# microsoft/YOLaT-VectorGraphicsRecognition

Hardware: AMD Instinct MI355X
Metric: graphs_per_sec (higher is better)
Workload: dtype f32

## Files before the change

yolat_vectorgraphicsrecognition_amd/csrc/common.hpp:

```cpp
#pragma once
#include <hip/hip_runtime.h>
#include <stdint.h>

#include "../../include/yolat_hip.h"

typedef float f32x16 __attribute__((ext_vector_type(16)));
typedef float f32x4 __attribute__((ext_vector_type(4)));

#define YL_LAUNCH_CHECK()                          \
  do {                                             \
    hipError_t e__ = hipGetLastError();            \
    if (e__ != hipSuccess) return (int)e__;        \
  } while (0)

static inline int yl_cdiv(long a, long b) { return (int)((a + b - 1) / b); }
static inline bool yl_aligned16(const void* p) { return (((uintptr_t)p) & 15) == 0; }
static inline bool yl_strict_fp32() {
  static int v = -1;
  if (v < 0) { const char* e = getenv("YOLAT_STRICT_FP32"); v = (e && e[0] == '1') ? 1 : 0; }
  return v != 0;
}

struct YlGate { const int* p; int val; };
__device__ __forceinline__ bool yl_gate_dead(const YlGate& g) { return g.p != nullptr && *g.p != g.val; }
// ... 542 lines not shown
    }
    __syncthreads();
  }

  static_assert(TM <= 2 && TN <= 2, "epilogue expansion covers up to 2x2 sub-tiles");
#define YL_EPI(i, j)                                                                                              \
  if constexpr ((i) < TM && (j) < TN)                                                                             \
    wave_epilogue(acc[i][j], row0 + wm * WM + (i) * 32, col0 + wn * WN + (j) * 32 + l31, lhi, ep, M, N, pre[i][j], \
                  smem + wave * (32 * YL_STAGE_LD));
  YL_EPI(0, 0) YL_EPI(0, 1) YL_EPI(1, 0) YL_EPI(1, 1)
#undef YL_EPI
}

template <int BM, int BN, int BK, class AL, class BL, bool B_NFAST>
__global__ void __launch_bounds__(256) k_gemm_nt(AL A, BL B, Epilogue ep, int M, int N, int K) {
  int rt_, ct_;
  yl_xcd_tile(rt_, ct_);
  gemm_nt_tile<BM, BN, BK, AL, BL, B_NFAST>(A, B, ep, M, N, K, rt_, ct_);
}

template <int BM, int BN, int BK, class AL, class BL>
__global__ void __launch_bounds__(256) k_gemm_nt_pair(AL A0, BL B0, Epilogue e0, AL A1, BL B1, Epilogue e1,
                                                      int M, int N, int K) {
  if (blockIdx.y == 0) gemm_nt_tile<BM, BN, BK, AL, BL, false>(A0, B0, e0, M, N, K, blockIdx.x, 0);
  else gemm_nt_tile<BM, BN, BK, AL, BL, false>(A1, B1, e1, M, N, K, blockIdx.x, 0);
}

static __global__ void __launch_bounds__(256) k_gemm_nt_two(DenseOp A0, DenseOp B0, Epilogue e0, int M0, int N0, int K0, int tm0,
                                                     int tn0, DenseOp A1, DenseOp B1, Epilogue e1, int M1, int N1,
                                                     int K1, int tm1, int tn1) {
  const int n1 = tm1 * tn1, n1p = (n1 + 7) & ~7;
  const int id = blockIdx.x;
  if (id < n1p) {
    if (id < n1) gemm_nt_tile<64, 64, 32, DenseOp, DenseOp, false>(A1, B1, e1, M1, N1, K1, id / tn1, id % tn1);
    return;
  }
  const int n0 = tm0 * tn0, j = id - n1p;
  const int chunk = n0 >> 3, rem = n0 & 7;
  const int xcd = j & 7, slot = j >> 3;
  const int logical = xcd * chunk + (xcd < rem ? xcd : rem) + slot;
  gemm_nt_tile<64, 64, 32, DenseOp, DenseOp, false>(A0, B0, e0, M0, N0, K0, logical / tn0, logical % tn0);
}

struct NodeUv {
  DenseOp af, wuv, wr, as, wn;
  Epilogue euv, er, en;
  int N, C, Cin;
};
int yl_build_node_uv(NodeUv* a, const float* f_in, int64_t ld_f, const float* s_in, int64_t ld_s, int64_t N,
                     int64_t Cin, const float* Wuv, const float* uv_bias, const float* Wr, const float* br,
                     const float* Wn, const float* bn, const float* sn, const float* tn, int64_t C, float* UV,
                     int64_t ld_uv, float* f_out, int64_t ld_fo, float* s_out, int64_t ld_so);
constexpr int N3_KMAX = 8, N3_ROWS = 32, N3_ITERS = 4;
template <int WAVES = 4, int ITERS = N3_ITERS>
__device__ __forceinline__ void node3_smallk_body(const NodeUv& a, int vb) {
  constexpr int ROWS = 8 * WAVES;
  __shared__ __attribute__((aligned(16))) float xs[ITERS][WAVES][2][64];
  const int lane = threadIdx.x & 63, wave = threadIdx.x >> 6;
  const int C = a.C, Cin = a.Cin, N = a.N;
  const int r0 = vb * (ROWS * ITERS), r1 = yl_min(r0 + ROWS * ITERS, N);
  const int c4 = 4 * lane;
  const int prob = c4 < 2 * C ? 0 : (c4 < 3 * C ? 1 : 2);
  const int col = prob == 0 ? c4 : (prob == 1 ? c4 - 2 * C : c4 - 3 * C);
  const int relu = prob == 0 ? a.euv.relu : (prob == 1 ? a.er.relu : a.en.relu);
  float* Y = prob == 0 ? a.euv.Y : (prob == 1 ? a.er.Y : a.en.Y);
  unsigned short* Yh = prob == 0 ? a.euv.Yh : (prob == 1 ? a.er.Yh : a.en.Yh);
  const long ldy = prob == 0 ? a.euv.ldy : (prob == 1 ? a.er.ldy : a.en.ldy);
  const int lu = lane >> 3, lk = lane & 7;
  float fa[ITERS], sa[ITERS];
#pragma unroll
  for (int it = 0; it < ITERS; ++it) {
    const long row = yl_min(r0 + ROWS * it + 8 * wave + lu, N - 1);
    const int kc = yl_min(lk, Cin - 1);
    const float f = a.af.p[row * a.af.ld + kc], g = a.as.p[row * a.as.ld + kc];
    fa[it] = lk < Cin ? f : 0.f;
    sa[it] = lk < Cin ? g : 0.f;
  }
  __shared__ __attribute__((aligned(16))) float wl[256][N3_KMAX];
  __shared__ float cl[3][256];
  if (threadIdx.x < 256) {
    const int t = threadIdx.x;
    const int tp = t < 2 * C ? 0 : (t < 3 * C ? 1 : 2);
    const int tc = tp == 0 ? t : (tp == 1 ? t - 2 * C : t - 3 * C);
    const float* __restrict__ twp = tp == 0 ? a.wuv.p : (tp == 1 ? a.wr.p : a.wn.p);
    const long tld = tp == 0 ? a.wuv.ld : (tp == 1 ? a.wr.ld : a.wn.ld);
    const float* tb = tp == 0 ? a.euv.bias : (tp == 1 ? a.er.bias : a.en.bias);
    const float* ts = tp == 0 ? a.euv.scale : (tp == 1 ? a.er.scale : a.en.scale);
    const float* th = tp == 0 ? a.euv.shift : (tp == 1 ? a.er.shift : a.en.shift);
    float wr_[N3_KMAX];
#pragma unroll
    for (int k = 0; k < N3_KMAX; ++k) wr_[k] = twp[(long)tc * tld + yl_min(k, Cin - 1)];
    const float vb_ = (tb ? tb : twp)[tb ? tc : 0], vs_ = (ts ? ts : twp)[ts ? tc : 0], vh_ = (ts ? th : twp)[ts ? tc : 0];
#pragma unroll
    for (int k = 0; k < N3_KMAX; ++k) wl[t][k] = k < Cin ? wr_[k] : 0.f;
    cl[0][t] = tb ? vb_ : 0.f;
    cl[1][t] = ts ? vs_ : 1.f;
    cl[2][t] = ts ? vh_ : 0.f;
  }
#pragma unroll
  for (int it = 0; it < ITERS; ++it) { xs[it][wave][0][lane] = fa[it]; xs[it][wave][1][lane] = sa[it]; }
  __syncthreads();
  float w[4][N3_KMAX], b[4], sc[4], sh[4];
#pragma unroll
  for (int j = 0; j < 4; ++j) {
    const float4 w0 = *reinterpret_cast<const float4*>(&wl[c4 + j][0]), w1 = *reinterpret_cast<const float4*>(&wl[c4 + j][4]);
    w[j][0] = w0.x; w[j][1] = w0.y; w[j][2] = w0.z; w[j][3] = w0.w;
    w[j][4] = w1.x; w[j][5] = w1.y; w[j][6] = w1.z; w[j][7] = w1.w;
    b[j] = cl[0][c4 + j]; sc[j] = cl[1][c4 + j]; sh[j] = cl[2][c4 + j];
  }
  const float floor = relu ? 0.f : -INFINITY;
#pragma unroll 1
  for (int it = 0; it < ITERS; ++it) {
    const float* mine = xs[it][wave][prob == 2 ? 1 : 0];
    const int rb = r0 + ROWS * it + 8 * wave;
    if (rb >= r1) break;
#pragma unroll
    for (int u = 0; u < 8; ++u) {
      const float4 x0 = *reinterpret_cast<const float4*>(mine + 8 * u);
      const float4 x1 = *reinterpret_cast<const float4*>(mine + 8 * u + 4);
      const float x[8] = {x0.x, x0.y, x0.z, x0.w, x1.x, x1.y, x1.z, x1.w};
      float v[4];
#pragma unroll
      for (int j = 0; j < 4; ++j) {
        float acc = 0.f;
#pragma unroll
        for (int k = 0; k < N3_KMAX; ++k) acc = fmaf(x[k], w[j][k], acc);
        v[j] = fmaxf(fmaf(acc + b[j], sc[j], sh[j]), floor);
      }
      const int row = rb + u;
      if (row < r1) {
        if (Yh != nullptr) {
          uint2 o;
          o.x = yl_pack_bf16(v[0], v[1]); o.y = yl_pack_bf16(v[2], v[3]);
          *reinterpret_cast<uint2*>(Yh + (long)row * ldy + col) = o;
        } else {
          *reinterpret_cast<float4*>(Y + (long)row * ldy + col) = make_float4(v[0], v[1], v[2], v[3]);
        }
      }
    }
  }
}

bool yl_node3_smallk_ok(const NodeUv& a);
bool yl_node3_smallk_shape_ok(const NodeUv& a);
int yl_node3_smallk(const NodeUv& a, hipStream_t st, YlGate gate = YlGate{nullptr, 0});
int yl_fusion_rows_x6_key64(const float* A, long lda, long N, long K, const float* W, const float* bias, long F,
                            const float* sgn, const int* node_seg, unsigned long long* keys, uint16_t* wsplit,
                            yolat_stream_t stream);
int yl_fusion_rows_bf16_key64(const float* A, long lda, long N, long K, const float* W, const float* bias, long F,
                              const float* sgn, const int* node_seg, unsigned long long* keys, uint16_t* wimg,
                              yolat_stream_t stream);
#define YL_POOL_ZERO 1
#define YL_POOL_MAX 2
#define YL_POOL_MEAN 4
struct PoolRider {
  const float* feats; const float* fsup; long ld; int D, F, P; const int* seg_ptr; float* Z; long ldz;
  int parts, blocks;
};
__device__ __forceinline__ void yl_pool_rider(const PoolRider& r, int vb, int nvb, int tid, int nthreads) {
  const int wz = (r.parts & YL_POOL_ZERO) ? r.F : 0, wx = (r.parts & YL_POOL_MAX) ? r.D : 0,
            wm = (r.parts & YL_POOL_MEAN) ? r.D : 0;
  const int W = wz + wx + wm;
  const long total = (long)r.P * W;
  for (long i = (long)vb * nthreads + tid; i < total; i += (long)nvb * nthreads) {
    const int p = (int)(i / W), c = (int)(i - (long)p * W);
    float* z = r.Z + (long)p * r.ldz;
    if (c < wz) { z[c] = 0.f; continue; }
    const bool is_max = c < wz + wx;
    const int k = is_max ? c - wz : c - wz - wx;
    const float* src = (is_max ? r.feats : r.fsup) + k;
    const int r0 = r.seg_ptr[p], r1 = r.seg_ptr[p + 1];
    float best = 0.f, sm = 0.f;
    bool any = false;
    int q = r0;
    for (; q + 8 <= r1; q += 8) {
      float v[8];
#pragma unroll
      for (int j = 0; j < 8; ++j) v[j] = src[(long)(q + j) * r.ld];
#pragma unroll
      for (int j = 0; j < 8; ++j) {
        if (!any || v[j] > best) { best = v[j]; any = true; }
        sm += v[j];
      }
    }
    for (; q < r1; ++q) {
      const float v = src[(long)q * r.ld];
      if (!any || v > best) { best = v; any = true; }
      sm += v;
    }
    if (is_max) z[r.F + k] = best;
    else {
      const int cnt = r1 - r0;
      z[2 * r.F + r.D + k] = sm / (float)(cnt > 1 ? cnt : 1);
// ... 443 lines not shown
```

yolat_vectorgraphicsrecognition_amd/csrc/graph.hip:

```cpp
#include "common.hpp"

__global__ void k_edge_count(const int64_t* edge, long se, long sc, int E, int N, int* src32,
                             int* dst32, int* cnt, int* status) {
  const int e = blockIdx.x * blockDim.x + threadIdx.x;
  if (e >= E) return;
  int64_t s = edge[(long)e * se];
  int64_t d = edge[(long)e * se + sc];
  if (s < 0 || s >= N || d < 0 || d >= N) {
    atomicOr(status, YOLAT_STATUS_EDGE_RANGE);
    s = s < 0 ? 0 : (s >= N ? N - 1 : s);
    d = d < 0 ? 0 : (d >= N ? N - 1 : d);
  }
  src32[e] = (int)s; dst32[e] = (int)d;
  atomicAdd(&cnt[d], 1);
}

__global__ void k_count32(const int* key, int n, int* cnt) {
  const int i = blockIdx.x * blockDim.x + threadIdx.x;
  if (i >= n) return;
  const int k = key[i];
  if (k >= 0) atomicAdd(&cnt[k], 1);
}

__global__ void __launch_bounds__(1024) k_scan_excl(int* cnt, int N, int* ptr) {
// ... 332 lines not shown
  const int d = dst32[e];
  items[local[d] + prep_prefix(btot, d / PREP_BLK) + rank[e]] = e;
}

__device__ __forceinline__ void prep_rows_body(int t, const int* local, const int* btot, int N, int E, const int* items,
                                               const int* src32, const int* dst32, const float4* attr, int* row_ptr,
                                               int* perm, int* src_csr, int* dst_csr, float4* attr_csr) {
  __shared__ int sh[PREP_OFFS + 4], wsum[4];
  const bool have = prep_offsets_lds(btot, (N + 1 + PREP_BLK - 1) / PREP_BLK, sh, wsum);
  auto off = [&](int i) { return local[i] + (have ? sh[i / PREP_BLK] : prep_prefix(btot, i / PREP_BLK)); };
  if (t <= N) row_ptr[t] = off(t);
  if (t >= E) return;
  const int e = items[t];
  const int i = dst32[e];
  const int b = off(i), en = off(i + 1);
  int r = 0;
  for (int j = b; j < en; j += 8) {
    int v[8];
#pragma unroll
    for (int k = 0; k < 8; ++k) v[k] = items[yl_min(j + k, en - 1)];
#pragma unroll
    for (int k = 0; k < 8; ++k) r += (j + k < en && v[k] < e) ? 1 : 0;
  }
  const int pos = b + r;
  const int sv = src32[e];
  const float4 av = attr[e];
  perm[pos] = e;
  src_csr[pos] = sv;
  dst_csr[pos] = i;
  attr_csr[pos] = av;
}

__global__ void __launch_bounds__(256) k_prep_rows(const int* local, const int* btot, int N, int E, const int* items,
                                                   const int* src32, const int* dst32, const float4* attr, int* row_ptr,
                                                   int* perm, int* src_csr, int* dst_csr, float4* attr_csr) {
  prep_rows_body(blockIdx.x * 256 + threadIdx.x, local, btot, N, E, items, src32, dst32, attr, row_ptr, perm, src_csr,
                 dst_csr, attr_csr);
}

template <int BK>
__global__ void __launch_bounds__(256) k_prep_rows_node3(const int* local, const int* btot, int N, int E,
                                                         const int* items, const int* src32, const int* dst32,
                                                         const float4* attr, int* row_ptr, int* perm, int* src_csr,
                                                         int* dst_csr, float4* attr_csr, int rows_blocks, NodeUv a) {
  if ((int)blockIdx.x < rows_blocks) {
    prep_rows_body(blockIdx.x * 256 + threadIdx.x, local, btot, N, E, items, src32, dst32, attr, row_ptr, perm, src_csr,
                   dst_csr, attr_csr);
    return;
  }
  const int t = blockIdx.x - rows_blocks;
  node_uv_tile<BK>(a, t >> 2, t & 3);
}

#define PS_T 1024
#define PS_NW (PS_T / 64)
#define PS_RMAX 256
#define PS_CAP 4096
#define PS_PF 8
#ifndef PS_NODE_ITERS
#define PS_NODE_ITERS 2
#endif
struct PrepSmall {
  const int64_t* edge; long se, sc; const float4* attr; const int64_t* bbox; long P;
  int E, N, R, nprep, nseg;
  int* row_ptr; int* perm; int* src_csr; int* dst_csr; float4* attr_csr; int* seg_ptr; int* node_seg; int* status;
};

__device__ __forceinline__ void ps_emit(const PrepSmall& g, int e, int d, int pos) {
  int64_t s = g.edge[(long)e * g.se];
  const float4 av = g.attr[e];
  if (s < 0 || s >= g.N) {
    atomicOr(g.status, YOLAT_STATUS_EDGE_RANGE);
    s = s < 0 ? 0 : g.N - 1;
  }
  g.perm[pos] = e;
  g.src_csr[pos] = (int)s;
  g.dst_csr[pos] = d;
  g.attr_csr[pos] = av;
}

template <int MODE>
__device__ __forceinline__ void ps_walk(const PrepSmall& g, int r0, int r1, int* rowcnt, int* cw, unsigned long long* mw,
                                        int* list_n, unsigned* list, int& below, int base, const int* rowstart) {
  const int lane = threadIdx.x & 63, w = threadIdx.x >> 6;
  const unsigned long long lt = (1ull << lane) - 1ull;
  const int per = ((g.E + PS_NW * 64 - 1) / (PS_NW * 64)) * 64;
  const int wb = w * per, we = yl_min(wb + per, g.E);
  for (int eb = wb; eb < we; eb += 64 * PS_PF) {
    int64_t dv[PS_PF];
#pragma unroll
    for (int j = 0; j < PS_PF; ++j) {
      const int e = yl_min(eb + 64 * j + lane, g.E - 1);
      dv[j] = g.edge[(long)e * g.se + g.sc];
    }
    if (MODE == 0) {
      unsigned long long om[PS_PF];
      int nown = 0;
#pragma unroll
      for (int j = 0; j < PS_PF; ++j) {
        const bool valid = eb + 64 * j + lane < we;
        const int d = dv[j] < 0 ? 0 : (dv[j] >= g.N ? g.N - 1 : (int)dv[j]);
        below += (valid && d < r0) ? 1 : 0;
        om[j] = __ballot(valid && d >= r0 && d < r1);
        nown += __popcll(om[j]);
      }
      if (nown == 0) continue;
      int s0 = 0;
      if (lane == 0) s0 = atomicAdd(list_n, nown);
      s0 = __builtin_amdgcn_readfirstlane(s0);
#pragma unroll
      for (int j = 0; j < PS_PF; ++j) {
        if ((om[j] >> lane) & 1ull) {
          const int dl = (dv[j] < 0 ? 0 : (dv[j] >= g.N ? g.N - 1 : (int)dv[j])) - r0, slot = s0 + __popcll(om[j] & lt);
          atomicAdd(&rowcnt[dl], 1);
          if (dv[j] < 0 || dv[j] >= g.N) atomicOr(g.status, YOLAT_STATUS_EDGE_RANGE);
          if (slot < PS_CAP) list[slot] = (unsigned)(eb + 64 * j + lane) | ((unsigned)dl << 20);
        }
        s0 += __popcll(om[j]);
      }
    } else {
#pragma unroll
      for (int j = 0; j < PS_PF; ++j) {
        const int e = eb + 64 * j + lane;
        const int d = dv[j] < 0 ? 0 : (dv[j] >= g.N ? g.N - 1 : (int)dv[j]);
        const bool own = e < we && d >= r0 && d < r1;
        if (__ballot(own) == 0ull) continue;
        const int dl = own ? d - r0 : 0;
        const int c = cw[dl];
        if (own) atomicOr(&mw[dl], 1ull << lane);
        const unsigned long long m = mw[dl];
        if (own && (m & lt) == 0ull) {
          cw[dl] = c + __popcll(m);
          mw[dl] = 0ull;
        }
        if (MODE == 2 && own) ps_emit(g, e, d, base + rowstart[dl] + c + __popcll(m & lt));
      }
    }
  }
}

__global__ void __launch_bounds__(PS_T) k_prep_small(PrepSmall g, NodeUv a, int with_node) {
  const int tid = threadIdx.x, lane = tid & 63, w = tid >> 6;
  if ((int)blockIdx.x >= g.nprep + g.nseg) {
    if (with_node) node3_smallk_body<PS_NW, PS_NODE_ITERS>(a, blockIdx.x - g.nprep - g.nseg);
    return;
  }
  if ((int)blockIdx.x >= g.nprep) {
    const int t = (blockIdx.x - g.nprep) * PS_T + tid;
    if (t > g.N) return;
    long prev = (t == 0) ? -1 : g.bbox[t - 1];
    long cur = (t == g.N) ? g.P : g.bbox[t];
    if (t < g.N) {
      if (cur < 0 || cur >= g.P) { atomicOr(g.status, YOLAT_STATUS_SEG_RANGE); cur = cur < 0 ? 0 : g.P - 1; }
      g.node_seg[t] = (int)cur;
    }
    if (prev >= g.P) prev = g.P - 1;
    if (prev < -1) prev = -1;
    if (cur < prev) atomicOr(g.status, YOLAT_STATUS_SEG_UNSORTED);
    else for (long p = prev + 1; p <= cur; ++p) g.seg_ptr[p] = t;
    return;
  }
  __shared__ unsigned long long pool[PS_NW * PS_RMAX + PS_NW * PS_RMAX / 2];
  static_assert(2 * PS_CAP * sizeof(unsigned) <= sizeof(unsigned long long) * PS_NW * PS_RMAX, "list + grp fit the mask area");
  unsigned* list = reinterpret_cast<unsigned*>(pool);
  unsigned* grp = list + PS_CAP;
  unsigned long long (*msk)[PS_RMAX] = reinterpret_cast<unsigned long long (*)[PS_RMAX]>(pool);
  int (*cnt)[PS_RMAX] = reinterpret_cast<int (*)[PS_RMAX]>(pool + PS_NW * PS_RMAX);
  __shared__ int rowcnt[PS_RMAX], cur[PS_RMAX], rowstart[PS_RMAX];
  __shared__ int wbelow[PS_NW], wtot[PS_RMAX / 64], list_n;
  const int r0 = blockIdx.x * g.R, r1 = yl_min(r0 + g.R, g.N);
  const bool last = (int)blockIdx.x == g.nprep - 1;
  if (tid < PS_RMAX) { rowcnt[tid] = 0; cur[tid] = 0; }
  if (tid == 0) list_n = 0;
  __syncthreads();
  int below = 0;
  ps_walk<0>(g, r0, r1, rowcnt, nullptr, nullptr, &list_n, list, below, 0, nullptr);
#pragma unroll
  for (int off = 32; off > 0; off >>= 1) below += __shfl_down(below, off);
  if (lane == 0) wbelow[w] = below;
  __syncthreads();
  const int rt = tid < PS_RMAX ? rowcnt[tid] : 0;
  int incl = rt;
#pragma unroll
  for (int off = 1; off < 64; off <<= 1) {
    const int nb = __shfl_up(incl, off);
    if (lane >= off) incl += nb;
  }
  if (tid < PS_RMAX && lane == 63) wtot[w] = incl;
  int base = 0;
#pragma unroll
  for (int v = 0; v < PS_NW; ++v) base += wbelow[v];
  const int n_list = list_n;
  __syncthreads();
  if (tid < PS_RMAX) {
    int off = 0;
#pragma unroll
    for (int v = 0; v < PS_RMAX / 64; ++v) off += (v < w) ? wtot[v] : 0;
    rowstart[tid] = off + incl - rt;
    if (r0 + tid < r1) g.row_ptr[r0 + tid] = base + off + incl - rt;
    if (last && tid == PS_RMAX - 1) g.row_ptr[g.N] = base + off + incl;
  }
  if (n_list <= PS_CAP) {
    static_assert(PS_CAP == 4 * PS_T, "four list entries per thread, spelled out");
    __syncthreads();
    for (int i = tid; i < n_list; i += PS_T) {
      const unsigned en = list[i];
      const int dl = (int)(en >> 20);
      grp[rowstart[dl] + atomicAdd(&cur[dl], 1)] = en;
    }
    __syncthreads();
    if (n_list > 0) {
      const int lastv = n_list - 1;
      auto emit_k = [&](int i, unsigned en, int64_t sv, float a0, float a1, float a2, float a3) {
        if (i >= n_list) return;
        const int dl = (int)(en >> 20), b = rowstart[dl], n = rowcnt[dl];
        int r = 0;
        for (int u = 0; u < n; ++u) r += (grp[b + u] < en) ? 1 : 0;
        if (sv < 0 || sv >= g.N) { atomicOr(g.status, YOLAT_STATUS_EDGE_RANGE); sv = sv < 0 ? 0 : g.N - 1; }
        const int pos = base + b + r;
        g.perm[pos] = (int)(en & 0xFFFFFu);
        g.src_csr[pos] = (int)sv;
        g.dst_csr[pos] = r0 + dl;
        g.attr_csr[pos] = make_float4(a0, a1, a2, a3);
      };
#define PS_G(k)                                                                        \
      const unsigned en##k = list[yl_min(tid + (k) * PS_T, lastv)];                    \
      const int64_t sx##k = g.edge[(long)(en##k & 0xFFFFFu) * g.se];                   \
      const float4 ax##k = g.attr[en##k & 0xFFFFFu];
      PS_G(0) PS_G(1) PS_G(2) PS_G(3)
#undef PS_G
      emit_k(tid, en0, sx0, ax0.x, ax0.y, ax0.z, ax0.w);
      emit_k(tid + PS_T, en1, sx1, ax1.x, ax1.y, ax1.z, ax1.w);
      emit_k(tid + 2 * PS_T, en2, sx2, ax2.x, ax2.y, ax2.z, ax2.w);
      emit_k(tid + 3 * PS_T, en3, sx3, ax3.x, ax3.y, ax3.z, ax3.w);
    }
  } else {
    __syncthreads();
    for (int i = tid; i < PS_NW * PS_RMAX; i += PS_T) { (&cnt[0][0])[i] = 0; (&msk[0][0])[i] = 0ull; }
    __syncthreads();
    int unused = 0;
    ps_walk<1>(g, r0, r1, nullptr, cnt[w], msk[w], nullptr, nullptr, unused, 0, nullptr);
    __syncthreads();
    if (tid < PS_RMAX) {
      int run = 0;
#pragma unroll
      for (int v = 0; v < PS_NW; ++v) { const int t = cnt[v][tid]; cnt[v][tid] = run; run += t; }
    }
    __syncthreads();
    ps_walk<2>(g, r0, r1, nullptr, cnt[w], msk[w], nullptr, nullptr, unused, base, rowstart);
  }
}

#define PS_PLAN_ROWS 100
#define PS_PLAN_EDGES (PS_CAP / 2)
#define PS_PLAN_GRID 250
static int prep_small_rows(int64_t N, int64_t E, int64_t other_blocks) {
  static const bool on = []() { const char* e = getenv("YOLAT_PREP_SMALL"); return !(e && e[0] == '0'); }();
  static const int forced = []() { const char* e = getenv("YOLAT_PREP_R"); const int r = e ? atoi(e) : 0;
                                   return (r >= 1 && r <= PS_RMAX) ? r : 0; }();
  if (!on || N <= 0 || E < 0 || E > 98304) return 0;
  if (forced) return forced;
  int64_t r_edges = E > 0 ? (int64_t)PS_PLAN_EDGES * N / E : PS_RMAX;
  if (r_edges < 1) r_edges = 1;
  int64_t R = PS_PLAN_ROWS;
  if (R > r_edges) R = r_edges;
  if (R > N) R = N;
  if ((N + R - 1) / R + other_blocks > PS_PLAN_GRID) {
    const int64_t room = PS_PLAN_GRID - other_blocks;
    if (room < 1) return 0;
    R = (N + room - 1) / room;
    if (R > PS_RMAX || R > r_edges) return 0;
  }
  return (int)R;
}

extern "C" int yolat_graph_prepare_plan(int64_t N, int64_t E, int64_t other_wgs, int32_t* rows, int32_t* csr_wgs) {
  const int R = (other_wgs < 0) ? 0 : prep_small_rows(N, E, other_wgs);
  if (rows) *rows = R;
  if (csr_wgs) *csr_wgs = R > 0 ? (int32_t)((N + R - 1) / R) : 0;
  return R > 0 ? 1 : 0;
}

extern "C" size_t yolat_graph_work_elems(int64_t N, int64_t E) {
  return (size_t)(2 * (((N + 1) + 63) / 64 * 64) + 4 * E + (N + 1) / PREP_BLK + 16);
}

int yl_graph_prepare_impl(const int64_t* edge, int64_t stride_e, int64_t stride_c, const float* e_attr,
                              const int64_t* bbox_idx, int64_t E, int64_t N, int64_t P, int32_t* row_ptr,
                              int32_t* perm, int32_t* src_csr, int32_t* dst_csr, float* attr_csr, int32_t* seg_ptr,
                              int32_t* node_seg, int32_t* work, int32_t* status, const NodeUv* extra, bool primed,
                              yolat_stream_t stream) {
  if (N <= 0 || E < 0 || N >= (1LL << 31) - 8192 || E >= (1LL << 31) - 256) return YOLAT_E_INVALID;
  if (!row_ptr || !work || !status) return YOLAT_E_INVALID;
  if (E > 0 && (!edge || !e_attr || !perm || !src_csr || !dst_csr || !attr_csr)) return YOLAT_E_INVALID;
  if (bbox_idx && (P <= 0 || !seg_ptr || !node_seg)) return YOLAT_E_INVALID;
  if (E > 0 && !yl_aligned16(e_attr)) return YOLAT_E_UNSUPPORTED;
  hipStream_t st = (hipStream_t)stream;
  const int n1 = (int)N + 1;
  const int nblk = yl_cdiv(n1, PREP_BLK);
  const int n1p = (n1 + 63) / 64 * 64;
  int* cnt = work;
  int* local = cnt + n1p;
  int* btot = local + n1p;
  int* src32 = btot + nblk + 1;
  int* dst32 = src32 + E;
  int* rank = dst32 + E;
  int* items = rank + E;
  const int node_blocks = extra ? yl_cdiv(extra->N, 8 * PS_NW * PS_NODE_ITERS) : 0;
  const int seg_blocks = bbox_idx ? yl_cdiv(N + 1, PS_T) : 0;
  const int Rs = (extra == nullptr || yl_node3_smallk_shape_ok(*extra)) ? prep_small_rows(N, E, node_blocks + seg_blocks) : 0;
  if (Rs > 0) {
    PrepSmall g;
    g.edge = edge; g.se = (long)stride_e; g.sc = (long)stride_c; g.attr = reinterpret_cast<const float4*>(e_attr);
    g.bbox = bbox_idx; g.P = (long)P; g.E = (int)E; g.N = (int)N; g.R = Rs; g.nprep = yl_cdiv(N, Rs);
    g.nseg = seg_blocks;
    g.row_ptr = row_ptr; g.perm = perm; g.src_csr = src_csr; g.dst_csr = dst_csr;
    g.attr_csr = reinterpret_cast<float4*>(attr_csr); g.seg_ptr = seg_ptr; g.node_seg = node_seg; g.status = status;
    NodeUv none{};
    hipLaunchKernelGGL(k_prep_small, dim3(g.nprep + g.nseg + node_blocks), dim3(PS_T), 0, st, g, extra ? *extra : none,
                       extra ? 1 : 0);
    YL_LAUNCH_CHECK();
    return 0;
  }
  if (!primed) {
    hipLaunchKernelGGL(k_zero_i32, dim3(yl_cdiv(n1p, 1024)), dim3(256), 0, st, cnt, n1p);
    YL_LAUNCH_CHECK();
  }
  const long nthreads = (E > N + 1) ? E : N + 1;
  hipLaunchKernelGGL(k_prep_count_win, dim3(yl_cdiv(nthreads, PCW_E)), dim3(PCW_T), 0, st, edge, (long)stride_e,
                     (long)stride_c, (int)E, (int)N, src32, dst32, rank, cnt, bbox_idx, (long)P, seg_ptr,
                     node_seg, status);
  YL_LAUNCH_CHECK();
  hipLaunchKernelGGL(k_prep_scan, dim3(nblk), dim3(1024), 0, st, cnt, n1, local, btot);
  YL_LAUNCH_CHECK();
  if (E > 0) {
    hipLaunchKernelGGL(k_prep_fill, dim3(yl_cdiv(E, 256)), dim3(256), 0, st, dst32, rank, (int)E, local, btot,
                       items);
    YL_LAUNCH_CHECK();
  }
  const int rows_blocks = yl_cdiv(E > n1 ? E : n1, 256);
  if (extra != nullptr && yl_node3_smallk_ok(*extra)) {
    hipLaunchKernelGGL(k_prep_rows, dim3(rows_blocks), dim3(256), 0, st, local, btot, (int)N, (int)E, items, src32, dst32,
                       reinterpret_cast<const float4*>(e_attr), row_ptr, perm, src_csr, dst_csr,
                       reinterpret_cast<float4*>(attr_csr));
    YL_LAUNCH_CHECK();
    return yl_node3_smallk(*extra, st);
  }
  if (extra != nullptr) {
    const unsigned total = (unsigned)rows_blocks + 4u * (unsigned)yl_cdiv(extra->N, 64);
    if (extra->Cin <= 16)
      hipLaunchKernelGGL(k_prep_rows_node3<16>, dim3(total), dim3(256), 0, st, local, btot, (int)N, (int)E, items, src32, dst32,
                         reinterpret_cast<const float4*>(e_attr), row_ptr, perm, src_csr, dst_csr,
                         reinterpret_cast<float4*>(attr_csr), rows_blocks, *extra);
    else
      hipLaunchKernelGGL(k_prep_rows_node3<32>, dim3(total), dim3(256), 0, st, local, btot, (int)N, (int)E, items, src32, dst32,
                         reinterpret_cast<const float4*>(e_attr), row_ptr, perm, src_csr, dst_csr,
                         reinterpret_cast<float4*>(attr_csr), rows_blocks, *extra);
  } else {
    hipLaunchKernelGGL(k_prep_rows, dim3(rows_blocks), dim3(256), 0, st, local, btot, (int)N, (int)E, items, src32, dst32,
                       reinterpret_cast<const float4*>(e_attr), row_ptr, perm, src_csr, dst_csr,
                       reinterpret_cast<float4*>(attr_csr));
  }
// ... 53 lines not shown
```

Baseline: 16120.

## Halve prep_small block size, share LDS pool, prefetch edge sources during scan

Cuts the fused small-graph prep kernel from 1024 to 512 threads and makes the node-transform path share one LDS pool with the CSR path, which should lower per-block LDS and raise occupancy. In the first edge walk it reads each (src,dst) pair as one 16-byte vector and keeps the sources in shared memory. It also issues the first batch of attribute and source gathers before the row-offset scan, so their latency overlaps the scan. Segment blocks now cover 1024 rows with a loop, and the emit step loops over batches instead of assuming four entries per thread. The risks are fewer threads per prep block and more LDS used per entry for the stored sources.

```diff
diff --git a/yolat_vectorgraphicsrecognition_amd/csrc/common.hpp b/yolat_vectorgraphicsrecognition_amd/csrc/common.hpp
--- a/yolat_vectorgraphicsrecognition_amd/csrc/common.hpp
+++ b/yolat_vectorgraphicsrecognition_amd/csrc/common.hpp
@@ -618,10 +618,12 @@
                      const float* Wn, const float* bn, const float* sn, const float* tn, int64_t C, float* UV,
                      int64_t ld_uv, float* f_out, int64_t ld_fo, float* s_out, int64_t ld_so);
 constexpr int N3_KMAX = 8, N3_ROWS = 32, N3_ITERS = 4;
+template <int WAVES, int ITERS>
+constexpr int N3_LDS_FLOATS() { return ITERS * WAVES * 2 * 64 + 256 * 8 + 3 * 256; }
 template <int WAVES = 4, int ITERS = N3_ITERS>
-__device__ __forceinline__ void node3_smallk_body(const NodeUv& a, int vb) {
+__device__ __forceinline__ void node3_smallk_rows(const NodeUv& a, int vb, float* lds) {
   constexpr int ROWS = 8 * WAVES;
-  __shared__ __attribute__((aligned(16))) float xs[ITERS][WAVES][2][64];
+  float (*xs)[WAVES][2][64] = reinterpret_cast<float (*)[WAVES][2][64]>(lds);
   const int lane = threadIdx.x & 63, wave = threadIdx.x >> 6;
   const int C = a.C, Cin = a.Cin, N = a.N;
   const int r0 = vb * (ROWS * ITERS), r1 = yl_min(r0 + ROWS * ITERS, N);
@@ -642,8 +644,8 @@
     fa[it] = lk < Cin ? f : 0.f;
     sa[it] = lk < Cin ? g : 0.f;
   }
-  __shared__ __attribute__((aligned(16))) float wl[256][N3_KMAX];
-  __shared__ float cl[3][256];
+  float (*wl)[N3_KMAX] = reinterpret_cast<float (*)[N3_KMAX]>(lds + ITERS * WAVES * 2 * 64);
+  float (*cl)[256] = reinterpret_cast<float (*)[256]>(lds + ITERS * WAVES * 2 * 64 + 256 * N3_KMAX);
   if (threadIdx.x < 256) {
     const int t = threadIdx.x;
     const int tp = t < 2 * C ? 0 : (t < 3 * C ? 1 : 2);
@@ -705,6 +707,12 @@
       }
     }
   }
+}
+template <int WAVES = 4, int ITERS = N3_ITERS>
+__device__ __forceinline__ void node3_smallk_body(const NodeUv& a, int vb) {
+  static_assert(N3_KMAX == 8, "N3_LDS_FLOATS counts 8 weights per column");
+  __shared__ __attribute__((aligned(16))) float lds[N3_LDS_FLOATS<WAVES, ITERS>()];
+  node3_smallk_rows<WAVES, ITERS>(a, vb, lds);
 }
 
 bool yl_node3_smallk_ok(const NodeUv& a);
diff --git a/yolat_vectorgraphicsrecognition_amd/csrc/graph.hip b/yolat_vectorgraphicsrecognition_amd/csrc/graph.hip
--- a/yolat_vectorgraphicsrecognition_amd/csrc/graph.hip
+++ b/yolat_vectorgraphicsrecognition_amd/csrc/graph.hip
@@ -408,14 +408,24 @@
   node_uv_tile<BK>(a, t >> 2, t & 3);
 }
 
-#define PS_T 1024
+#ifndef PS_T
+#define PS_T 512
+#endif
 #define PS_NW (PS_T / 64)
 #define PS_RMAX 256
 #define PS_CAP 4096
+#ifndef PS_PF
 #define PS_PF 8
+#endif
+#ifndef PS_TAIL
+#define PS_TAIL 1
+#endif
+#define PS_EB 4
+#define PS_SEG_ROWS 1024
 #ifndef PS_NODE_ITERS
-#define PS_NODE_ITERS 2
+#define PS_NODE_ITERS (256 / (8 * PS_NW))
 #endif
+static_assert(PS_T == 512 || PS_T == 1024, "k_prep_small: 8 or 16 waves");
 struct PrepSmall {
   const int64_t* edge; long se, sc; const float4* attr; const int64_t* bbox; long P;
   int E, N, R, nprep, nseg;
@@ -435,19 +445,27 @@
   g.attr_csr[pos] = av;
 }
 
-template <int MODE>
+template <int MODE, bool VEC>
 __device__ __forceinline__ void ps_walk(const PrepSmall& g, int r0, int r1, int* rowcnt, int* cw, unsigned long long* mw,
-                                        int* list_n, unsigned* list, int& below, int base, const int* rowstart) {
+                                        int* list_n, unsigned* list, int* srcs, int& below, int base,
+                                        const int* rowstart) {
+  static_assert(!VEC || MODE == 0, "the ordered walks read the destinations only");
   const int lane = threadIdx.x & 63, w = threadIdx.x >> 6;
   const unsigned long long lt = (1ull << lane) - 1ull;
   const int per = ((g.E + PS_NW * 64 - 1) / (PS_NW * 64)) * 64;
   const int wb = w * per, we = yl_min(wb + per, g.E);
   for (int eb = wb; eb < we; eb += 64 * PS_PF) {
-    int64_t dv[PS_PF];
+    int64_t dv[PS_PF], sv[VEC ? PS_PF : 1];
 #pragma unroll
     for (int j = 0; j < PS_PF; ++j) {
       const int e = yl_min(eb + 64 * j + lane, g.E - 1);
-      dv[j] = g.edge[(long)e * g.se + g.sc];
+      if (VEC) {
+        const longlong2 row = reinterpret_cast<const longlong2*>(g.edge)[e];
+        sv[VEC ? j : 0] = row.x;
+        dv[j] = row.y;
+      } else {
+        dv[j] = g.edge[(long)e * g.se + g.sc];
+      }
     }
     if (MODE == 0) {
       unsigned long long om[PS_PF];
@@ -469,8 +487,12 @@
         if ((om[j] >> lane) & 1ull) {
           const int dl = (dv[j] < 0 ? 0 : (dv[j] >= g.N ? g.N - 1 : (int)dv[j])) - r0, slot = s0 + __popcll(om[j] & lt);
           atomicAdd(&rowcnt[dl], 1);
-          if (dv[j] < 0 || dv[j] >= g.N) atomicOr(g.status, YOLAT_STATUS_EDGE_RANGE);
-          if (slot < PS_CAP) list[slot] = (unsigned)(eb + 64 * j + lane) | ((unsigned)dl << 20);
+          const int64_t s = VEC ? sv[VEC ? j : 0] : 0;
+          if (dv[j] < 0 || dv[j] >= g.N || s < 0 || s >= g.N) atomicOr(g.status, YOLAT_STATUS_EDGE_RANGE);
+          if (slot < PS_CAP) {
+            list[slot] = (unsigned)(eb + 64 * j + lane) | ((unsigned)dl << 20);
+            if (VEC) srcs[slot] = s < 0 ? 0 : (s >= g.N ? g.N - 1 : (int)s);
+          }
         }
         s0 += __popcll(om[j]);
       }
@@ -497,44 +519,73 @@
 
 __global__ void __launch_bounds__(PS_T) k_prep_small(PrepSmall g, NodeUv a, int with_node) {
   const int tid = threadIdx.x, lane = tid & 63, w = tid >> 6;
+  constexpr int PS_POOL_LIST = (2 + PS_TAIL) * PS_CAP * (int)sizeof(unsigned), PS_POOL_ORD = PS_NW * PS_RMAX * 12;
+  constexpr int PS_POOL_NODE = N3_LDS_FLOATS<PS_NW, PS_NODE_ITERS>() * (int)sizeof(float);
+  constexpr int PS_POOL_CSR = PS_POOL_LIST > PS_POOL_ORD ? PS_POOL_LIST : PS_POOL_ORD;
+  __shared__ __attribute__((aligned(16))) unsigned long long pool[(PS_POOL_CSR > PS_POOL_NODE ? PS_POOL_CSR : PS_POOL_NODE) / 8];
   if ((int)blockIdx.x >= g.nprep + g.nseg) {
-    if (with_node) node3_smallk_body<PS_NW, PS_NODE_ITERS>(a, blockIdx.x - g.nprep - g.nseg);
+    if (with_node) node3_smallk_rows<PS_NW, PS_NODE_ITERS>(a, blockIdx.x - g.nprep - g.nseg, reinterpret_cast<float*>(pool));
     return;
   }
   if ((int)blockIdx.x >= g.nprep) {
-    const int t = (blockIdx.x - g.nprep) * PS_T + tid;
-    if (t > g.N) return;
-    long prev = (t == 0) ? -1 : g.bbox[t - 1];
-    long cur = (t == g.N) ? g.P : g.bbox[t];
-    if (t < g.N) {
-      if (cur < 0 || cur >= g.P) { atomicOr(g.status, YOLAT_STATUS_SEG_RANGE); cur = cur < 0 ? 0 : g.P - 1; }
-      g.node_seg[t] = (int)cur;
-    }
-    if (prev >= g.P) prev = g.P - 1;
-    if (prev < -1) prev = -1;
-    if (cur < prev) atomicOr(g.status, YOLAT_STATUS_SEG_UNSORTED);
-    else for (long p = prev + 1; p <= cur; ++p) g.seg_ptr[p] = t;
+#pragma unroll
+    for (int k = 0; k < PS_SEG_ROWS / PS_T; ++k) {
+      const int t = (blockIdx.x - g.nprep) * PS_SEG_ROWS + k * PS_T + tid;
+      if (t > g.N) continue;
+      long prev = (t == 0) ? -1 : g.bbox[t - 1];
+      long cur = (t == g.N) ? g.P : g.bbox[t];
+      if (t < g.N) {
+        if (cur < 0 || cur >= g.P) { atomicOr(g.status, YOLAT_STATUS_SEG_RANGE); cur = cur < 0 ? 0 : g.P - 1; }
+        g.node_seg[t] = (int)cur;
+      }
+      if (prev >= g.P) prev = g.P - 1;
+      if (prev < -1) prev = -1;
+      if (cur < prev) atomicOr(g.status, YOLAT_STATUS_SEG_UNSORTED);
+      else for (long p = prev + 1; p <= cur; ++p) g.seg_ptr[p] = t;
+    }
     return;
   }
-  __shared__ unsigned long long pool[PS_NW * PS_RMAX + PS_NW * PS_RMAX / 2];
-  static_assert(2 * PS_CAP * sizeof(unsigned) <= sizeof(unsigned long long) * PS_NW * PS_RMAX, "list + grp fit the mask area");
   unsigned* list = reinterpret_cast<unsigned*>(pool);
   unsigned* grp = list + PS_CAP;
+  int* srcs = reinterpret_cast<int*>(grp + PS_CAP);
   unsigned long long (*msk)[PS_RMAX] = reinterpret_cast<unsigned long long (*)[PS_RMAX]>(pool);
   int (*cnt)[PS_RMAX] = reinterpret_cast<int (*)[PS_RMAX]>(pool + PS_NW * PS_RMAX);
   __shared__ int rowcnt[PS_RMAX], cur[PS_RMAX], rowstart[PS_RMAX];
   __shared__ int wbelow[PS_NW], wtot[PS_RMAX / 64], list_n;
   const int r0 = blockIdx.x * g.R, r1 = yl_min(r0 + g.R, g.N);
   const bool last = (int)blockIdx.x == g.nprep - 1;
+  const bool vec = PS_TAIL && g.se == 2 && g.sc == 1 && (reinterpret_cast<uintptr_t>(g.edge) & 15) == 0;
   if (tid < PS_RMAX) { rowcnt[tid] = 0; cur[tid] = 0; }
   if (tid == 0) list_n = 0;
   __syncthreads();
   int below = 0;
-  ps_walk<0>(g, r0, r1, rowcnt, nullptr, nullptr, &list_n, list, below, 0, nullptr);
+  if (vec) ps_walk<0, PS_TAIL != 0>(g, r0, r1, rowcnt, nullptr, nullptr, &list_n, list, srcs, below, 0, nullptr);
+  else ps_walk<0, false>(g, r0, r1, rowcnt, nullptr, nullptr, &list_n, list, nullptr, below, 0, nullptr);
 #pragma unroll
   for (int off = 32; off > 0; off >>= 1) below += __shfl_down(below, off);
   if (lane == 0) wbelow[w] = below;
   __syncthreads();
+  const int n_list = list_n;
+  unsigned en0 = 0, en1 = 0, en2 = 0, en3 = 0;
+  int64_t sx0 = 0, sx1 = 0, sx2 = 0, sx3 = 0;
+  float4 ax0 = make_float4(0.f, 0.f, 0.f, 0.f), ax1 = ax0, ax2 = ax0, ax3 = ax0;
+  static_assert(PS_EB == 4, "the batch is spelled out");
+#define PS_G(k, b0)                                                                    \
+  const int at##k = yl_min((b0) + tid + (k) * PS_T, n_list - 1);                       \
+  en##k = list[at##k];
+#define PS_GATHER(b0)                                                                  \
+  {                                                                                    \
+    PS_G(0, b0) PS_G(1, b0) PS_G(2, b0) PS_G(3, b0)                                    \
+    if (vec) { sx0 = srcs[at0]; sx1 = srcs[at1]; sx2 = srcs[at2]; sx3 = srcs[at3]; }   \
+    ax0 = g.attr[en0 & 0xFFFFFu]; ax1 = g.attr[en1 & 0xFFFFFu];                        \
+    ax2 = g.attr[en2 & 0xFFFFFu]; ax3 = g.attr[en3 & 0xFFFFFu];                        \
+    if (!vec) {                                                                        \
+      sx0 = g.edge[(long)(en0 & 0xFFFFFu) * g.se]; sx1 = g.edge[(long)(en1 & 0xFFFFFu) * g.se];  \
+      sx2 = g.edge[(long)(en2 & 0xFFFFFu) * g.se]; sx3 = g.edge[(long)(en3 & 0xFFFFFu) * g.se];  \
+    }                                                                                  \
+  }
+  const bool listp = n_list > 0 && n_list <= PS_CAP;
+  if (PS_TAIL && listp) PS_GATHER(0)
   const int rt = tid < PS_RMAX ? rowcnt[tid] : 0;
   int incl = rt;
 #pragma unroll
@@ -546,7 +597,6 @@
   int base = 0;
 #pragma unroll
   for (int v = 0; v < PS_NW; ++v) base += wbelow[v];
-  const int n_list = list_n;
   __syncthreads();
   if (tid < PS_RMAX) {
     int off = 0;
@@ -557,45 +607,40 @@
     if (last && tid == PS_RMAX - 1) g.row_ptr[g.N] = base + off + incl;
   }
   if (n_list <= PS_CAP) {
-    static_assert(PS_CAP == 4 * PS_T, "four list entries per thread, spelled out");
     __syncthreads();
     for (int i = tid; i < n_list; i += PS_T) {
-      const unsigned en = list[i];
-      const int dl = (int)(en >> 20);
-      grp[rowstart[dl] + atomicAdd(&cur[dl], 1)] = en;
-    }
-    __syncthreads();
-    if (n_list > 0) {
-      const int lastv = n_list - 1;
-      auto emit_k = [&](int i, unsigned en, int64_t sv, float a0, float a1, float a2, float a3) {
-        if (i >= n_list) return;
-        const int dl = (int)(en >> 20), b = rowstart[dl], n = rowcnt[dl];
-        int r = 0;
-        for (int u = 0; u < n; ++u) r += (grp[b + u] < en) ? 1 : 0;
-        if (sv < 0 || sv >= g.N) { atomicOr(g.status, YOLAT_STATUS_EDGE_RANGE); sv = sv < 0 ? 0 : g.N - 1; }
-        const int pos = base + b + r;
-        g.perm[pos] = (int)(en & 0xFFFFFu);
-        g.src_csr[pos] = (int)sv;
-        g.dst_csr[pos] = r0 + dl;
-        g.attr_csr[pos] = make_float4(a0, a1, a2, a3);
-      };
-#define PS_G(k)                                                                        \
-      const unsigned en##k = list[yl_min(tid + (k) * PS_T, lastv)];                    \
-      const int64_t sx##k = g.edge[(long)(en##k & 0xFFFFFu) * g.se];                   \
-      const float4 ax##k = g.attr[en##k & 0xFFFFFu];
-      PS_G(0) PS_G(1) PS_G(2) PS_G(3)
+      const unsigned e = list[i];
+      const int dl = (int)(e >> 20);
+      grp[rowstart[dl] + atomicAdd(&cur[dl], 1)] = e;
+    }
+    __syncthreads();
+    auto emit_k = [&](int i, unsigned e, int64_t sv, float a0, float a1, float a2, float a3) {
+      if (i >= n_list) return;
+      const int dl = (int)(e >> 20), b = rowstart[dl], n = rowcnt[dl];
+      int r = 0;
+      for (int u = 0; u < n; ++u) r += (grp[b + u] < e) ? 1 : 0;
+      if (sv < 0 || sv >= g.N) { atomicOr(g.status, YOLAT_STATUS_EDGE_RANGE); sv = sv < 0 ? 0 : g.N - 1; }
+      const int pos = base + b + r;
+      g.perm[pos] = (int)(e & 0xFFFFFu);
+      g.src_csr[pos] = (int)sv;
+      g.dst_csr[pos] = r0 + dl;
+      g.attr_csr[pos] = make_float4(a0, a1, a2, a3);
+    };
+    for (int b0 = 0; b0 < n_list; b0 += PS_EB * PS_T) {
+      if (!PS_TAIL || b0 > 0) PS_GATHER(b0)
+      emit_k(b0 + tid, en0, sx0, ax0.x, ax0.y, ax0.z, ax0.w);
+      emit_k(b0 + tid + PS_T, en1, sx1, ax1.x, ax1.y, ax1.z, ax1.w);
+      emit_k(b0 + tid + 2 * PS_T, en2, sx2, ax2.x, ax2.y, ax2.z, ax2.w);
+      emit_k(b0 + tid + 3 * PS_T, en3, sx3, ax3.x, ax3.y, ax3.z, ax3.w);
+    }
+#undef PS_GATHER
 #undef PS_G
-      emit_k(tid, en0, sx0, ax0.x, ax0.y, ax0.z, ax0.w);
-      emit_k(tid + PS_T, en1, sx1, ax1.x, ax1.y, ax1.z, ax1.w);
-      emit_k(tid + 2 * PS_T, en2, sx2, ax2.x, ax2.y, ax2.z, ax2.w);
-      emit_k(tid + 3 * PS_T, en3, sx3, ax3.x, ax3.y, ax3.z, ax3.w);
-    }
   } else {
     __syncthreads();
     for (int i = tid; i < PS_NW * PS_RMAX; i += PS_T) { (&cnt[0][0])[i] = 0; (&msk[0][0])[i] = 0ull; }
     __syncthreads();
     int unused = 0;
-    ps_walk<1>(g, r0, r1, nullptr, cnt[w], msk[w], nullptr, nullptr, unused, 0, nullptr);
+    ps_walk<1, false>(g, r0, r1, nullptr, cnt[w], msk[w], nullptr, nullptr, nullptr, unused, 0, nullptr);
     __syncthreads();
     if (tid < PS_RMAX) {
       int run = 0;
@@ -603,7 +648,7 @@
       for (int v = 0; v < PS_NW; ++v) { const int t = cnt[v][tid]; cnt[v][tid] = run; run += t; }
     }
     __syncthreads();
-    ps_walk<2>(g, r0, r1, nullptr, cnt[w], msk[w], nullptr, nullptr, unused, base, rowstart);
+    ps_walk<2, false>(g, r0, r1, nullptr, cnt[w], msk[w], nullptr, nullptr, nullptr, unused, base, rowstart);
   }
 }
 
@@ -663,7 +708,7 @@
   int* rank = dst32 + E;
   int* items = rank + E;
   const int node_blocks = extra ? yl_cdiv(extra->N, 8 * PS_NW * PS_NODE_ITERS) : 0;
-  const int seg_blocks = bbox_idx ? yl_cdiv(N + 1, PS_T) : 0;
+  const int seg_blocks = bbox_idx ? yl_cdiv(N + 1, PS_SEG_ROWS) : 0;
   const int Rs = (extra == nullptr || yl_node3_smallk_shape_ok(*extra)) ? prep_small_rows(N, E, node_blocks + seg_blocks) : 0;
   if (Rs > 0) {
     PrepSmall g;
```

Measured after the change: 16480, median of 6. +2.2%, better.

## Add lean node3 path, interleave prep edge scan, and raise prep kernel occupancy

Applied to the files above, without the earlier changes.

Adds a LEAN variant of the small-K node body in which each wave handles contiguous rows. It walks a single output pointer, reloads scale and shift from LDS per row instead of keeping them in registers, and adds scheduling barriers to cut register pressure. The MODE 0 edge walk in k_prep_small now strides edges across waves in an interleaved way so reads are coalesced, and it computes the clamped destination and range flag once. The kernel gets launch_bounds(PS_T, 8) plus a static assert that two workgroups' LDS fit one CU. The aim is higher occupancy and less redundant work, with a risk of extra LDS reads or register spills under the tighter bound.

```diff
diff --git a/yolat_vectorgraphicsrecognition_amd/csrc/common.hpp b/yolat_vectorgraphicsrecognition_amd/csrc/common.hpp
--- a/yolat_vectorgraphicsrecognition_amd/csrc/common.hpp
+++ b/yolat_vectorgraphicsrecognition_amd/csrc/common.hpp
@@ -618,7 +618,11 @@
                      const float* Wn, const float* bn, const float* sn, const float* tn, int64_t C, float* UV,
                      int64_t ld_uv, float* f_out, int64_t ld_fo, float* s_out, int64_t ld_so);
 constexpr int N3_KMAX = 8, N3_ROWS = 32, N3_ITERS = 4;
-template <int WAVES = 4, int ITERS = N3_ITERS>
+template <int WAVES, int ITERS>
+constexpr size_t node3_smallk_lds_bytes() {
+  return sizeof(float) * (size_t)(ITERS * WAVES * 2 * 64 + 256 * N3_KMAX + 3 * 256);
+}
+template <int WAVES = 4, int ITERS = N3_ITERS, bool LEAN = false>
 __device__ __forceinline__ void node3_smallk_body(const NodeUv& a, int vb) {
   constexpr int ROWS = 8 * WAVES;
   __shared__ __attribute__((aligned(16))) float xs[ITERS][WAVES][2][64];
@@ -636,14 +640,14 @@
   float fa[ITERS], sa[ITERS];
 #pragma unroll
   for (int it = 0; it < ITERS; ++it) {
-    const long row = yl_min(r0 + ROWS * it + 8 * wave + lu, N - 1);
+    const long row = yl_min((LEAN ? r0 + 8 * (ITERS * wave + it) : r0 + ROWS * it + 8 * wave) + lu, N - 1);
     const int kc = yl_min(lk, Cin - 1);
     const float f = a.af.p[row * a.af.ld + kc], g = a.as.p[row * a.as.ld + kc];
     fa[it] = lk < Cin ? f : 0.f;
     sa[it] = lk < Cin ? g : 0.f;
   }
   __shared__ __attribute__((aligned(16))) float wl[256][N3_KMAX];
-  __shared__ float cl[3][256];
+  __shared__ __attribute__((aligned(16))) float cl[3][256];
   if (threadIdx.x < 256) {
     const int t = threadIdx.x;
     const int tp = t < 2 * C ? 0 : (t < 3 * C ? 1 : 2);
@@ -672,9 +676,56 @@
     const float4 w0 = *reinterpret_cast<const float4*>(&wl[c4 + j][0]), w1 = *reinterpret_cast<const float4*>(&wl[c4 + j][4]);
     w[j][0] = w0.x; w[j][1] = w0.y; w[j][2] = w0.z; w[j][3] = w0.w;
     w[j][4] = w1.x; w[j][5] = w1.y; w[j][6] = w1.z; w[j][7] = w1.w;
-    b[j] = cl[0][c4 + j]; sc[j] = cl[1][c4 + j]; sh[j] = cl[2][c4 + j];
+    b[j] = cl[0][c4 + j];
+    if (!LEAN) { sc[j] = cl[1][c4 + j]; sh[j] = cl[2][c4 + j]; }
   }
   const float floor = relu ? 0.f : -INFINITY;
+  if constexpr (LEAN) {
+    const bool half = Yh != nullptr;
+    const long pitch = ldy * (half ? 2 : 4);
+    const int wv = __builtin_amdgcn_readfirstlane(wave);
+    const float* mine = &xs[0][0][prob == 2 ? 1 : 0][0] + wv * (2 * 64);
+    const int rw = r0 + 8 * ITERS * wv;
+    char* yp = (half ? reinterpret_cast<char*>(Yh + col) : reinterpret_cast<char*>(Y + col)) + (long)rw * pitch;
+#pragma unroll 1
+    for (int it = 0; it < ITERS; ++it) {
+      const int rb = rw + 8 * it;
+      if (rb >= r1) break;
+      asm volatile("" : "+v"(yp));
+#pragma unroll
+      for (int u = 0; u < 8; ++u) {
+        asm volatile("" ::: "memory");
+        const float4 x0 = *reinterpret_cast<const float4*>(mine + 8 * u);
+        const float4 x1 = *reinterpret_cast<const float4*>(mine + 8 * u + 4);
+        const float x[8] = {x0.x, x0.y, x0.z, x0.w, x1.x, x1.y, x1.z, x1.w};
+        float acc[4];
+#pragma unroll
+        for (int j = 0; j < 4; ++j) {
+          acc[j] = 0.f;
+#pragma unroll
+          for (int k = 0; k < N3_KMAX; ++k) acc[j] = fmaf(x[k], w[j][k], acc[j]);
+        }
+        __builtin_amdgcn_sched_barrier(0);
+        const float4 s4 = *reinterpret_cast<const float4*>(&cl[1][c4]), h4 = *reinterpret_cast<const float4*>(&cl[2][c4]);
+        const float scv[4] = {s4.x, s4.y, s4.z, s4.w}, shv[4] = {h4.x, h4.y, h4.z, h4.w};
+        float v[4];
+#pragma unroll
+        for (int j = 0; j < 4; ++j) v[j] = fmaxf(fmaf(acc[j] + b[j], scv[j], shv[j]), floor);
+        if (rb + u < r1) {
+          if (half) {
+            uint2 o;
+            o.x = yl_pack_bf16(v[0], v[1]); o.y = yl_pack_bf16(v[2], v[3]);
+            *reinterpret_cast<uint2*>(yp) = o;
+          } else {
+            *reinterpret_cast<float4*>(yp) = make_float4(v[0], v[1], v[2], v[3]);
+          }
+        }
+        yp += pitch;
+      }
+      mine += WAVES * 2 * 64;
+    }
+    return;
+  }
 #pragma unroll 1
   for (int it = 0; it < ITERS; ++it) {
     const float* mine = xs[it][wave][prob == 2 ? 1 : 0];
diff --git a/yolat_vectorgraphicsrecognition_amd/csrc/graph.hip b/yolat_vectorgraphicsrecognition_amd/csrc/graph.hip
--- a/yolat_vectorgraphicsrecognition_amd/csrc/graph.hip
+++ b/yolat_vectorgraphicsrecognition_amd/csrc/graph.hip
@@ -440,24 +440,25 @@
                                         int* list_n, unsigned* list, int& below, int base, const int* rowstart) {
   const int lane = threadIdx.x & 63, w = threadIdx.x >> 6;
   const unsigned long long lt = (1ull << lane) - 1ull;
-  const int per = ((g.E + PS_NW * 64 - 1) / (PS_NW * 64)) * 64;
-  const int wb = w * per, we = yl_min(wb + per, g.E);
-  for (int eb = wb; eb < we; eb += 64 * PS_PF) {
-    int64_t dv[PS_PF];
-#pragma unroll
-    for (int j = 0; j < PS_PF; ++j) {
-      const int e = yl_min(eb + 64 * j + lane, g.E - 1);
-      dv[j] = g.edge[(long)e * g.se + g.sc];
-    }
-    if (MODE == 0) {
+  if (MODE == 0) {
+    for (int eb = 64 * w; eb < g.E; eb += 64 * PS_NW * PS_PF) {
+      int64_t dv[PS_PF];
+#pragma unroll
+      for (int j = 0; j < PS_PF; ++j) {
+        const int e = yl_min(eb + 64 * PS_NW * j + lane, g.E - 1);
+        dv[j] = g.edge[(long)e * g.se + g.sc];
+      }
+      int d[PS_PF];
+      unsigned bad = 0u;
       unsigned long long om[PS_PF];
       int nown = 0;
 #pragma unroll
       for (int j = 0; j < PS_PF; ++j) {
-        const bool valid = eb + 64 * j + lane < we;
-        const int d = dv[j] < 0 ? 0 : (dv[j] >= g.N ? g.N - 1 : (int)dv[j]);
-        below += (valid && d < r0) ? 1 : 0;
-        om[j] = __ballot(valid && d >= r0 && d < r1);
+        const bool valid = eb + 64 * PS_NW * j + lane < g.E;
+        bad |= (dv[j] < 0 || dv[j] >= g.N) ? (1u << j) : 0u;
+        d[j] = dv[j] < 0 ? 0 : (dv[j] >= g.N ? g.N - 1 : (int)dv[j]);
+        below += (valid && d[j] < r0) ? 1 : 0;
+        om[j] = __ballot(valid && d[j] >= r0 && d[j] < r1);
         nown += __popcll(om[j]);
       }
       if (nown == 0) continue;
@@ -467,14 +468,26 @@
 #pragma unroll
       for (int j = 0; j < PS_PF; ++j) {
         if ((om[j] >> lane) & 1ull) {
-          const int dl = (dv[j] < 0 ? 0 : (dv[j] >= g.N ? g.N - 1 : (int)dv[j])) - r0, slot = s0 + __popcll(om[j] & lt);
+          const int dl = d[j] - r0, slot = s0 + __popcll(om[j] & lt);
           atomicAdd(&rowcnt[dl], 1);
-          if (dv[j] < 0 || dv[j] >= g.N) atomicOr(g.status, YOLAT_STATUS_EDGE_RANGE);
-          if (slot < PS_CAP) list[slot] = (unsigned)(eb + 64 * j + lane) | ((unsigned)dl << 20);
+          if ((bad >> j) & 1u) atomicOr(g.status, YOLAT_STATUS_EDGE_RANGE);
+          if (slot < PS_CAP) list[slot] = (unsigned)(eb + 64 * PS_NW * j + lane) | ((unsigned)dl << 20);
         }
         s0 += __popcll(om[j]);
       }
-    } else {
+    }
+    return;
+  }
+  const int per = ((g.E + PS_NW * 64 - 1) / (PS_NW * 64)) * 64;
+  const int wb = w * per, we = yl_min(wb + per, g.E);
+  for (int eb = wb; eb < we; eb += 64 * PS_PF) {
+    int64_t dv[PS_PF];
+#pragma unroll
+    for (int j = 0; j < PS_PF; ++j) {
+      const int e = yl_min(eb + 64 * j + lane, g.E - 1);
+      dv[j] = g.edge[(long)e * g.se + g.sc];
+    }
+    {
 #pragma unroll
       for (int j = 0; j < PS_PF; ++j) {
         const int e = eb + 64 * j + lane;
@@ -495,14 +508,13 @@
   }
 }
 
-__global__ void __launch_bounds__(PS_T) k_prep_small(PrepSmall g, NodeUv a, int with_node) {
-  const int tid = threadIdx.x, lane = tid & 63, w = tid >> 6;
+__global__ void __launch_bounds__(PS_T, 8) k_prep_small(PrepSmall g, NodeUv a, int with_node) {
   if ((int)blockIdx.x >= g.nprep + g.nseg) {
-    if (with_node) node3_smallk_body<PS_NW, PS_NODE_ITERS>(a, blockIdx.x - g.nprep - g.nseg);
+    if (with_node) node3_smallk_body<PS_NW, PS_NODE_ITERS, true>(a, blockIdx.x - g.nprep - g.nseg);
     return;
   }
   if ((int)blockIdx.x >= g.nprep) {
-    const int t = (blockIdx.x - g.nprep) * PS_T + tid;
+    const int t = (blockIdx.x - g.nprep) * PS_T + threadIdx.x;
     if (t > g.N) return;
     long prev = (t == 0) ? -1 : g.bbox[t - 1];
     long cur = (t == g.N) ? g.P : g.bbox[t];
@@ -516,6 +528,9 @@
     else for (long p = prev + 1; p <= cur; ++p) g.seg_ptr[p] = t;
     return;
   }
+  int tid = threadIdx.x;
+  asm volatile("" : "+v"(tid));
+  const int lane = tid & 63, w = tid >> 6;
   __shared__ unsigned long long pool[PS_NW * PS_RMAX + PS_NW * PS_RMAX / 2];
   static_assert(2 * PS_CAP * sizeof(unsigned) <= sizeof(unsigned long long) * PS_NW * PS_RMAX, "list + grp fit the mask area");
   unsigned* list = reinterpret_cast<unsigned*>(pool);
@@ -524,6 +539,9 @@
   int (*cnt)[PS_RMAX] = reinterpret_cast<int (*)[PS_RMAX]>(pool + PS_NW * PS_RMAX);
   __shared__ int rowcnt[PS_RMAX], cur[PS_RMAX], rowstart[PS_RMAX];
   __shared__ int wbelow[PS_NW], wtot[PS_RMAX / 64], list_n;
+  static_assert(2 * (sizeof(pool) + sizeof(rowcnt) + sizeof(cur) + sizeof(rowstart) + sizeof(wbelow) + sizeof(wtot) + 16 +
+                     node3_smallk_lds_bytes<PS_NW, PS_NODE_ITERS>()) <= 160 * 1024,
+                "two workgroups' LDS (this role's + the node-side role's) fit one CU");
   const int r0 = blockIdx.x * g.R, r1 = yl_min(r0 + g.R, g.N);
   const bool last = (int)blockIdx.x == g.nprep - 1;
   if (tid < PS_RMAX) { rowcnt[tid] = 0; cur[tid] = 0; }
```

Measured after the change: 16190 before, 16280 after (median of 3 runs). No clear change (+0.5%).
